# SandroMartens/DBGSOM

Hardware: NVIDIA B200
Metric: training samples/sec/epoch (higher is better)
Workload: dtype f16 tensor cores (tcgen05) + f64 re-score / f64 update / f64 smoothing

## Files before the change

### dbgsom_b200/_native.py

```python

from __future__ import annotations

import ctypes as C
import os

_LIB = None
LIB_NAME = "libdbgsom_b200.so"
LIB_PATH = os.path.join(os.path.dirname(os.path.abspath(__file__)), LIB_NAME)

ABI_VERSION = 10
COLSTATS_PARTS = 256
SELECT_OFF, SELECT_FLAG, SELECT_REFINE = 0, 1, 2
MAX_CAND = 8
BMU_SIMT = 0
BMU_TENSOR = 1
HOPS_MAX_M = 28000

c_void_p, c_int, c_int32, c_int64, c_size_t, c_float, c_double = (
    C.c_void_p, C.c_int, C.c_int32, C.c_int64, C.c_size_t, C.c_float, C.c_double,
)


class BmuArgs(C.Structure):
    _fields_ = [
        ("d_X", c_void_p),
# ... 88 lines not shown
        [c_void_p, c_int64, c_int, c_int64, c_void_p, c_float, c_void_p, c_void_p, c_int64, c_void_p, c_void_p],
    ),
    "dbgsom_prepare_x16_sorted": (
        c_int,
        [c_void_p, c_int64, c_int, c_int64, c_void_p, c_float, c_void_p, c_void_p, c_void_p, c_int64, c_void_p, c_void_p],
    ),
    "dbgsom_bmu_select_supported": (c_int, [c_int64, c_int64, c_int32, c_int32, c_int32]),
    "dbgsom_accumulate_perm_offset": (c_size_t, [c_int64, c_int32]),
    "dbgsom_prepare_w": (
        c_int,
        [c_void_p, c_int, c_int, c_void_p, c_float, c_void_p, c_void_p, c_void_p, c_int64, c_int, c_void_p,
         c_void_p, c_void_p, c_void_p, c_void_p],
    ),
    "dbgsom_exclude_duplicates": (c_int, [c_void_p, c_int, c_int, c_void_p, c_void_p, c_void_p, c_void_p]),
    "dbgsom_tile_bounds": (
        c_int, [c_void_p, c_int, c_int, c_void_p, c_float, c_void_p, c_void_p, c_int, c_void_p, c_void_p]
    ),
    "dbgsom_prepare_bias": (c_int, [c_void_p, c_int, c_void_p, c_void_p, c_void_p, c_void_p]),
    "dbgsom_bmu_workspace_bytes": (c_size_t, [c_int64, c_int32]),
    "dbgsom_bmu": (c_int, [C.POINTER(BmuArgs), c_void_p]),
    "dbgsom_bmu_candidates": (c_int, [C.POINTER(BmuArgs), c_void_p]),
    "dbgsom_bmu_resolve": (c_int, [C.POINTER(BmuArgs), c_void_p]),
    "dbgsom_accumulate_workspace_bytes": (c_size_t, [c_int64, c_int32, c_int32]),
    "dbgsom_accumulate": (c_int, [C.POINTER(AccumulateArgs), c_void_p]),
    "dbgsom_accumulate_weighted": (c_int, [C.POINTER(AccumulateArgs), c_void_p, c_void_p, c_void_p]),
    "dbgsom_smooth_workspace_bytes": (c_size_t, [c_int32, c_int32]),
    "dbgsom_smooth": (c_int, [C.POINTER(SmoothArgs), c_void_p]),
    "dbgsom_apply_row_ops": (c_int, [c_void_p, c_int, c_void_p, c_int, c_void_p]),
    "dbgsom_gather_rows": (c_int, [c_void_p, c_int64, c_int, c_void_p, c_int, c_void_p, c_void_p]),
    "dbgsom_node_stats": (
        c_int, [c_void_p, c_int32, c_void_p, c_int32, c_int64, c_void_p, c_int32, c_double, c_void_p, c_void_p]
# ... 57 lines not shown
```

### dbgsom_b200/csrc/bmu_tc.cu

```cuda
#include <cuda.h>

#include <cstdio>
#include <cstdlib>

#include "common.cuh"

namespace dbgsom {

namespace {

constexpr int BM = 128;
constexpr int BK = 64;
constexpr int UMMA_K = 16;
constexpr int A_TILE_BYTES = BM * BK * 2;
constexpr int EPI_WARP0 = 4;
constexpr int EPI_SUBS = 4;
constexpr int EPI_WARPS = 4 * EPI_SUBS;
constexpr int EPI_THREADS = EPI_WARPS * 32;
constexpr int TC_THREADS = (EPI_WARP0 + EPI_WARPS) * 32;
constexpr int KSUB = 4;
constexpr int MAX_RES_KB = 4;
constexpr int kFlagMaxCols = 4096;
constexpr int kFlagChunkBytes = kFlagMaxCols / 32 * BM * 4;

// ... 265 lines not shown
  static constexpr int RING_STAGE_BYTES = STAGES * STAGE_UNIT;
  static constexpr int SMEM_BYTES = RES_BYTES + RING_STAGE_BYTES + RING_BYTES + MISC_BYTES + WN_BYTES + EXTRA_BYTES + 1024;
  static constexpr int TMEM_COLS = ATM ? 512 : NACC * BN;
  static_assert(STAGES >= 2, "not enough shared memory for a pipeline");
};

struct Barriers {
  uint64_t full[16], empty[16];
  uint64_t a_full, a_empty;
  uint64_t tmem_full[4], tmem_empty[4];
  uint32_t tmem_base;
  EpiConst epi;
};

constexpr float kTileBoundFloor = 0.125f;
template <int NPASS, int NB, int BN, int RES_KB, int AKB, int CL, bool PAIR = false, int SEL = 0, bool TB = false,
          int SGT = 0>
__global__ void __launch_bounds__(TC_THREADS, 1)
    bmu_cand_tensor_kernel(const __grid_constant__ CUtensorMap map_xh, const __grid_constant__ CUtensorMap map_xl,
                           const __grid_constant__ CUtensorMap map_wh, const __grid_constant__ CUtensorMap map_wl,
                           const __grid_constant__ CUtensorMap map_wb, const float* __restrict__ bias_scale,
                           int64_t N, int KB, int NT, const float* __restrict__ wnorm,
                           const int32_t* __restrict__ proto_of_col, int pstride, int ties_any,
                           const float* __restrict__ xnorm16,
                           const float* __restrict__ wmax, float bound_coef, float acc_coef,
                           int32_t* __restrict__ idx_out, int32_t* __restrict__ cand_idx,
                           uint8_t* __restrict__ cand_count, const int32_t* __restrict__ row_perm,
                           unsigned long long* __restrict__ tile_mask,
                           int fg_shift, unsigned long long* __restrict__ sel_stats,
                           const float* __restrict__ tile_bound) {
// ... 383 lines not shown
    }
    const uint32_t epi_const_addr = smem_u32(&bars->epi);
    constexpr int CHUNKS = BN / 32;
    constexpr float kInf = 3.0e38f;
    if (sub == 0) row_min[t] = kInf;
    const int mpad = NT * BN;
    const bool wn_in_smem = !bias_mode && C::WN_SMEM_FLOATS > 0 && mpad <= C::WN_SMEM_FLOATS;
    if (wn_in_smem)
      for (int i = threadIdx.x - EPI_WARP0 * 32; i < mpad; i += EPI_THREADS) wn_smem[i] = wnorm[i];
    const float* wn_src = wn_in_smem ? wn_smem : wnorm;
    asm volatile("bar.sync 1, %0;" ::"n"(EPI_THREADS));
    uint32_t acc = 0, acc_phase = 0;
    uint32_t eph = 0;
    (void)eph;
    if constexpr (SEL == 1) {
      uint32_t* cta_mask = reinterpret_cast<uint32_t*>(sub_state);
      float* sub_min = reinterpret_cast<float*>(sub_state) + 4;
      if (threadIdx.x == EPI_WARP0 * 32) cta_mask[0] = cta_mask[1] = 0u;
      asm volatile("bar.sync 1, %0;" ::"n"(EPI_THREADS));
      const int n_chunks = NT * CHUNKS;
      for (int64_t it = 0; it < n_iters; ++it) {
        const int64_t row = tile_of(it) * BM + t;
        const bool valid = row < N;
        const int64_t orow = valid ? (row_perm ? (int64_t)row_perm[row] : row) : 0;
        const float tau = valid ? 2.f * tensor_score_bound(xnorm16[orow], wmax, bound_coef, acc_coef) : 0.f;
        float m1 = kInf;
        for (int nt = 0; nt < NT; ++nt) {
          mbar_wait(&bars->tmem_full[acc], acc_phase);
          tc_fence_after();
          const uint32_t tmem_acc = tmem_base + lane_base + acc * BN;
#pragma unroll 1
          for (int c = (sub - nt * CHUNKS) & (EPI_SUBS - 1); c < CHUNKS; c += EPI_SUBS) {
            uint32_t r[32];
            tmem_ld_32x32(tmem_acc + c * 32, r);
            float a1;
            if (bias_mode) {
              tmem_ld_wait();
              float gmx[8];
#pragma unroll
              for (int g = 0; g < 8; ++g)
                gmx[g] = fmaxf(fmaxf(__uint_as_float(r[4 * g + 0]), __uint_as_float(r[4 * g + 1])),
// ... 9 lines not shown
              tmem_ld_wait();
              float gmn[8];
#pragma unroll
              for (int g = 0; g < 8; ++g) {
                const float s0 = fmaf(-2.f, __uint_as_float(r[4 * g + 0]), w4[g].x);
                const float s1 = fmaf(-2.f, __uint_as_float(r[4 * g + 1]), w4[g].y);
                const float s2 = fmaf(-2.f, __uint_as_float(r[4 * g + 2]), w4[g].z);
                const float s3 = fmaf(-2.f, __uint_as_float(r[4 * g + 3]), w4[g].w);
                gmn[g] = fminf(fminf(s0, s1), fminf(s2, s3));
              }
              a1 = fminf(fminf(fminf(gmn[0], gmn[1]), fminf(gmn[2], gmn[3])),
                         fminf(fminf(gmn[4], gmn[5]), fminf(gmn[6], gmn[7])));
            }
            chunk_min[(nt * CHUNKS + c) * BM + t] = a1;
            m1 = fminf(m1, a1);
          }
          tc_fence_before();
          __syncwarp();
          if (lane == 0) mbar_arrive_cluster(mapa_u32(smem_u32(&bars->tmem_empty[acc]), 0));
          if (++acc == NACC) {
            acc = 0;
            acc_phase ^= 1;
          }
        }
        sub_min[t * EPI_SUBS + sub] = m1;
        asm volatile("bar.sync 1, %0;" ::"n"(EPI_THREADS));
        const float4 sm4 = *reinterpret_cast<const float4*>(sub_min + t * EPI_SUBS);
        const float thr = fminf(fminf(sm4.x, sm4.y), fminf(sm4.z, sm4.w)) + tau;
        uint32_t mlo = 0u, mhi = 0u;
        if (valid) {
          for (int ch = sub; ch < n_chunks; ch += EPI_SUBS) {
            const uint32_t bit = (uint32_t)(ch * 32) >> fg_shift;
            const uint32_t inb = chunk_min[ch * BM + t] <= thr ? 1u : 0u;
            mlo |= bit < 32u ? inb << bit : 0u;
            mhi |= bit >= 32u ? inb << (bit - 32u) : 0u;
          }
        }
        mlo = __reduce_or_sync(kFullMask, mlo);
        mhi = __reduce_or_sync(kFullMask, mhi);
        if (lane == 0) {
          if (mlo) atomicOr(&cta_mask[0], mlo);
          if (mhi) atomicOr(&cta_mask[1], mhi);
        }
        asm volatile("bar.sync 1, %0;" ::"n"(EPI_THREADS));
        if (threadIdx.x == EPI_WARP0 * 32) {
          const unsigned long long m64 = (unsigned long long)cta_mask[0] | ((unsigned long long)cta_mask[1] << 32);
          const int64_t pr = pair_of(it);
          if (m64 && pr < n_pairs) atomicOr(tile_mask + pr, m64);
          cta_mask[0] = cta_mask[1] = 0u;
        }
        asm volatile("bar.sync 1, %0;" ::"n"(EPI_THREADS));
      }
    } else {
    auto fetch_orow = [&](int64_t it_) -> int64_t {
      const int64_t r_ = it_ < n_iters ? tile_of(it_) * BM + t : N;
      return r_ < N ? (row_perm ? (int64_t)row_perm[r_] : r_) : -1;
    };
    auto fetch_mask = [&](int64_t it_) -> unsigned long long { return it_ < n_iters ? sel_mask(it_) : 0ull; };
    int64_t orow_n1 = fetch_orow(0);
    int64_t orow_n2 = fetch_orow(1);
    float xn_n1 = orow_n1 >= 0 ? xnorm16[orow_n1] : 0.f;
    unsigned long long mask_n1 = fetch_mask(0);
    for (int64_t it = 0; it < n_iters; ++it) {
      const int64_t row = tile_of(it) * BM + t;
      const int64_t orow = orow_n1 >= 0 ? orow_n1 : 0;
      const float tau = row < N ? 2.f * tensor_score_bound(xn_n1, wmax, bound_coef, acc_coef) : 0.f;
      const float xn_row = row < N ? xn_n1 : 0.f;
      unsigned long long selm = mask_n1;
      orow_n1 = orow_n2;
      xn_n1 = orow_n1 >= 0 ? xnorm16[orow_n1] : 0.f;
      orow_n2 = fetch_orow(it + 2);
      mask_n1 = fetch_mask(it + 1);
      float m1 = kInf, m2 = kInf, thr = kInf, evicted = __int_as_float(0x7f800000);
      float gate = __int_as_float(0x7f800000);
      asm volatile("st.shared.v4.f32 [%0], {%1,%1,%1,%1};" ::"r"(my_val_addr), "f"(gate) : "memory");
      asm volatile("st.shared.v4.s32 [%0], {%1,%1,%1,%1};" ::"r"(my_idx_addr), "r"(0x7fffffff) : "memory");
      const int n_sel = SEL == 2 ? __popcll(selm) : NT;
      for (int ti = 0; ti < n_sel; ++ti) {
        int nt = ti;
        if (SEL == 2) {
          nt = __ffsll((long long)selm) - 1;
          selm &= selm - 1;
        }
        float kb = 0.f;
        if (TB) {
          const float* tb = tile_bound + 2 * (nt * (BN / 128));
          float um = tb[0], wm = tb[1];
#pragma unroll
          for (int q = 1; q < BN / 128; ++q) {
            um = fmaxf(um, tb[2 * q]);
            wm = fmaxf(wm, tb[2 * q + 1]);
          }
          um = fmaxf(um, kTileBoundFloor * wmax[0]);
          wm = fmaxf(wm, kTileBoundFloor * wmax[2]);
          const float xw = xn_row * um;
          kb = xw * bound_coef + acc_coef * (xw + wm);
        }
// ... 24 lines not shown
              for (int e = 0; e < 16; ++e) {
                q0[e] = __float_as_uint(__uint_as_float(q0[e]) + __uint_as_float(p0[e]));
                q1[e] = __float_as_uint(__uint_as_float(q1[e]) + __uint_as_float(p1[e]));
              }
              tmem_st_32x16(qa, q0);
              tmem_st_32x16(qa + 16, q1);
            }
            tmem_st_wait();
          }
        } else {
          mbar_wait(&bars->tmem_full[acc], acc_phase);
        }
        tc_fence_after();
        const uint32_t tmem_acc = tmem_base + lane_base + acc * BN;
#pragma unroll 1
        for (int c = (sub - ti * CHUNKS) & (EPI_SUBS - 1); c < CHUNKS; c += EPI_SUBS) {
          uint32_t r[32];
          if (SEGM) {
            float sum[32];
            const int nseg = (KB + SEG - 1) / SEG;
            for (int seg = 0; seg < nseg; ++seg) {
              if (seg > 0) {
                mbar_wait(&bars->tmem_full[acc], acc_phase);
                tc_fence_after();
              }
              tmem_ld_32x32(tmem_base + lane_base + acc * BN + c * 32, r);
              tmem_ld_wait();
#pragma unroll
              for (int e = 0; e < 32; ++e) sum[e] = seg == 0 ? __uint_as_float(r[e]) : sum[e] + __uint_as_float(r[e]);
              if (seg < nseg - 1) {
                tc_fence_before();
// ... 295 lines not shown
      }
    }
    if (max_grid > (int64_t)max_clusters * CL) max_grid = (int64_t)max_clusters * CL;
  }
  if (grid > max_grid) grid = max_grid;
  cfg.gridDim = dim3((unsigned)grid);
  const float coef = tensor_bound_coef(NPASS, a.bound_scale);
  const float acc_coef = tensor_acc_coef_args(a);
  const int pstride = a.proto_stride > 0 && a.Mpad <= 65535 && a.proto_stride < a.Mpad ? a.proto_stride : 0;
  DBGSOM_CUDA_TRY(cudaLaunchKernelEx(&cfg, kern, mxh, mxl, mwh, mwl, mwb, with_bias ? a.d_bias_scale : (const float*)nullptr,
                                     a.N, KB, NT, a.d_wnorm, a.d_proto_of_col, pstride,
                                     a.n_bmu == 1 ? a.ties_any : 0, a.d_xnorm16, a.d_wmax, coef, acc_coef, a.d_idx, ws.cand_idx, ws.cand_count,
                                     a.d_row_perm, reinterpret_cast<unsigned long long*>(a.d_tile_mask),
                                     a.select_granule == 64 ? 6 : 7,
                                     a.d_stats ? reinterpret_cast<unsigned long long*>(a.d_stats) + 4 : (unsigned long long*)nullptr,
                                     TB ? a.d_tile_bound : (const float*)nullptr));
  DBGSOM_LAUNCH_CHECK();
  return DBGSOM_OK;
}

int cluster_size() {
  static int cl = 0;
  if (cl == 0) {
    const char* e = getenv("DBGSOM_TC_CLUSTER");
    cl = e ? atoi(e) : 2;
    if (cl != 1 && cl != 2 && cl != 4) cl = 2;
  }
  return cl;
}

template <int NPASS, int NB, int BN, int RES_KB, int AKB = 0>
// ... 19 lines not shown
  static const bool pairs = getenv("DBGSOM_TC_PAIR") == nullptr || atoi(getenv("DBGSOM_TC_PAIR")) != 0;
  return a.backend == DBGSOM_BMU_TENSOR && a.n_pass == 3 && a.ld16 / BK > MAX_RES_KB && pairs && cluster_size() >= 2 &&
         ceil_div<int64_t>(a.N, BM) >= sm_count();
}
int streamed_segm_mode() {
  static const int mode = getenv("DBGSOM_TC_SEGM") == nullptr ? 3 : atoi(getenv("DBGSOM_TC_SEGM"));
  return mode;
}
bool streamed_segmented(const dbgsom_bmu_args& a) { return streamed_segm_mode() == 1 && streamed_pairs(a); }
int streamed_tmem_sums(const dbgsom_bmu_args& a) {
  const int mode = streamed_segm_mode();
  return (mode == 2 || mode == 3) && streamed_pairs(a) ? (mode == 2 ? 8 : 4) : 0;
}
}
bool tile_bounds_active(const dbgsom_bmu_args& a) {
  return a.d_tile_bound != nullptr && a.n_bmu == 1 && a.select == DBGSOM_SELECT_OFF && streamed_pairs(a);
}
namespace {

template <int NPASS, int NB>
int launch_shape(const dbgsom_bmu_args& a, const BmuWorkspace& ws, cudaStream_t s) {
  const int KB = (int)(a.ld16 / BK);
  if constexpr (NPASS == 1) {
    if (KB <= 2) return launch_cfg<NPASS, NB, 256, 2>(a, ws, s);
    if (KB <= MAX_RES_KB) return launch_cfg<NPASS, NB, 256, 4>(a, ws, s);
    return launch_cfg<NPASS, NB, 256, 0>(a, ws, s);
  } else {
    static const bool a_smem = getenv("DBGSOM_TC_A_SMEM") != nullptr;
    if (KB <= 2) return a_smem ? launch_cfg<NPASS, NB, 128, 2>(a, ws, s) : launch_cfg<NPASS, NB, 128, 0, 2>(a, ws, s);
    if (KB <= MAX_RES_KB)
      return a_smem ? launch_cfg<NPASS, NB, 128, 4>(a, ws, s) : launch_cfg<NPASS, NB, 128, 0, 4>(a, ws, s);
// ... 80 lines not shown
```

### dbgsom_b200/csrc/capi.cu

```cuda
#include "common.cuh"

namespace dbgsom {
int run_colstats(const float*, int64_t, int, int64_t, const float*, const double*, double*, cudaStream_t);
int run_prepare_x16(const float*, int64_t, int, int64_t, const float*, float, const int32_t*, uint16_t*, uint16_t*, int64_t,
                    float*, cudaStream_t);
size_t accumulate_perm_offset(int64_t, int);
bool bmu_select_supported(int64_t N, int64_t ld16, int Mpad, int n_bmu, int granule);
int run_prepare_w(const double*, int, int, const float*, float, float*, uint16_t*, uint16_t*, int64_t, int,
                  const int32_t*, float*, double*, float*, cudaStream_t);
int run_exclude_duplicates(const double*, int, int, const int32_t*, float*, unsigned long long*, cudaStream_t);
int run_tile_bounds(const double*, int, int, const double*, float, const int32_t*, const float*, int, float*, cudaStream_t);
int run_prepare_bias(const float*, int, const float*, uint16_t*, float*, cudaStream_t);
int run_row_ops(double*, int, const int32_t*, int, cudaStream_t);
int run_gather_rows(const float*, int64_t, int, const int64_t*, int, double*, cudaStream_t);
size_t accumulate_workspace_bytes(int64_t, int, int);
int run_accumulate(const dbgsom_accumulate_args&, const double*, double*, cudaStream_t);
size_t label_hist_weighted_workspace_bytes(int64_t, int);
int run_label_counts_weighted(const int32_t*, const int32_t*, const double*, int64_t, int, int, double*, void*, cudaStream_t);
size_t smooth_workspace_bytes(int, int);
int run_smooth(const dbgsom_smooth_args&, cudaStream_t);
int run_node_stats(const int32_t*, int, const double*, int, int64_t, const int32_t*, int, double, const double*, double*,
                   cudaStream_t);
int run_label_hist(const int32_t*, int, const int32_t*, const double*, int64_t, int64_t, int, int, int32_t*, int64_t*,
                   cudaStream_t);
int run_umatrix(const double*, int, int, int64_t, const double*, double*, cudaStream_t);
int run_hops(const int32_t*, int, uint16_t*, int64_t, cudaStream_t);
// ... 97 lines not shown
  }
  if (a->D % 4 != 0 || a->ldx % 4 != 0 || !aligned16(a->d_X) || !aligned16(a->d_W32) || !aligned16(a->d_W))
    return DBGSOM_E_UNSUPPORTED;
  if (a->workspace_bytes < BmuWorkspace::bytes(a->N)) return DBGSOM_E_WORKSPACE;
  return DBGSOM_OK;
}

int dbgsom_exclude_duplicates(const double* d_W, int M, int D, const int32_t* d_col_of_proto, float* d_wnorm,
                              uint64_t* d_hash, void* stream) {
  if (!d_W || !d_wnorm || !d_hash || M <= 0 || D <= 0) return DBGSOM_E_BADARG;
  return run_exclude_duplicates(d_W, M, D, d_col_of_proto, d_wnorm, reinterpret_cast<unsigned long long*>(d_hash),
                                as_stream(stream));
}

int dbgsom_tile_bounds(const double* d_W, int M, int D, const double* d_wshift, float scale,
                       const int32_t* d_proto_of_col, const float* d_wnorm, int Mpad, float* d_tile_bound, void* stream) {
  if (!d_W || !d_wshift || !d_wnorm || !d_tile_bound || M <= 0 || D <= 0 || Mpad < M) return DBGSOM_E_BADARG;
  if (Mpad % 128 != 0) return DBGSOM_E_UNSUPPORTED;
  return run_tile_bounds(d_W, M, D, d_wshift, scale, d_proto_of_col, d_wnorm, Mpad, d_tile_bound, as_stream(stream));
}

int dbgsom_prepare_bias(const float* d_wnorm, int Mpad, const float* d_wmax, uint16_t* d_Wb16, float* d_bias_scale,
                        void* stream) {
  if (!d_wnorm || !d_wmax || !d_Wb16 || !d_bias_scale || Mpad <= 0) return DBGSOM_E_BADARG;
  return run_prepare_bias(d_wnorm, Mpad, d_wmax, d_Wb16, d_bias_scale, as_stream(stream));
}

int dbgsom_bmu_candidates(const dbgsom_bmu_args* a, void* stream) {
  const int rc = check_bmu_args(a);
  if (rc != DBGSOM_OK) return rc;
  const BmuWorkspace ws = BmuWorkspace::carve(a->d_workspace, a->N);
  if (a->backend == DBGSOM_BMU_SIMT) return launch_bmu_cand_simt(*a, ws, as_stream(stream));
  return launch_bmu_cand_tensor(*a, ws, as_stream(stream));
}
// ... 128 lines not shown
```

### dbgsom_b200/csrc/common.cuh

```cuda
#pragma once

#include <cuda_fp16.h>
#include <cuda_runtime.h>
#include <stdint.h>

#include <cmath>
#include <cstdlib>

#include "../../include/dbgsom_b200.h"

#define DBGSOM_CUDA_TRY(expr)                  \
  do {                                         \
    cudaError_t _e = (expr);                   \
    if (_e != cudaSuccess) return (int)_e;     \
  } while (0)

#define DBGSOM_LAUNCH_CHECK()                  \
  do {                                         \
    cudaError_t _e = cudaGetLastError();       \
    if (_e != cudaSuccess) return (int)_e;     \
  } while (0)

namespace dbgsom {

// ... 145 lines not shown
  }
};

__device__ __forceinline__ float tensor_score_bound(float xnorm, const float* __restrict__ wmax, float coef, float acc_coef) {
  const float xw = xnorm * wmax[0];
  return xw * coef + acc_coef * (xw + wmax[2]);
}
inline float tensor_acc_coef(int n_pass, int64_t ld16, int strict) {
  const double steps = (double)(ld16 / 16) * (n_pass == 3 ? 3.0 : 1.0);
  double c = 2.4e-7 * (steps > 48.0 ? (strict ? steps / 48.0 : sqrt(steps / 48.0)) : 1.0);
  if (const char* e = getenv("DBGSOM_ACC_SCALE")) c *= atof(e);
  return (float)c;
}
float tensor_acc_coef_args(const dbgsom_bmu_args& a);
bool tile_bounds_active(const dbgsom_bmu_args& a);
__host__ __device__ inline float tensor_bound_coef(int n_pass, float bound_scale) {
  if (n_pass == 1) return (bound_scale > 0.f ? bound_scale : 0.25f) * 1.953125e-3f;
  return (bound_scale > 0.f ? bound_scale : 0.0625f) * 1.9073486e-6f;
}

struct BmuWorkspace {
  int32_t* cand_idx;
  uint8_t* cand_count;
  int32_t* rescan_count;
  int32_t* rescan_rows;
  __host__ static size_t bytes(int64_t N) {
    return round_up<size_t>((size_t)N * kMaxCand * sizeof(int32_t), 256) + round_up<size_t>((size_t)N, 256) + 256 +
           round_up<size_t>((size_t)N * sizeof(int32_t), 256);
  }
  __host__ static BmuWorkspace carve(void* base, int64_t N) {
// ... 19 lines not shown
```

### dbgsom_b200/csrc/prep.cu

```cuda
#include "common.cuh"

namespace dbgsom {

namespace {

constexpr int CS_COLS = 32, CS_ROWS = 8;
template <bool WGT>
__global__ void __launch_bounds__(CS_COLS * CS_ROWS) colstats_kernel(const float* __restrict__ X, int64_t N, int D,
                                                                    int64_t ldx, const float* __restrict__ shift,
                                                                    const double* __restrict__ weight,
                                                                    double* __restrict__ moments,
                                                                    int64_t rows_per_block) {
  __shared__ double s1[CS_ROWS][CS_COLS], s2[CS_ROWS][CS_COLS], s3[CS_ROWS][CS_COLS];
  const int cx = threadIdx.x % CS_COLS, ry = threadIdx.x / CS_COLS;
  const int d = blockIdx.x * CS_COLS + cx;
  const int64_t r0 = (int64_t)blockIdx.y * rows_per_block;
  const int64_t r1 = r0 + rows_per_block < N ? r0 + rows_per_block : N;
  double a1 = 0.0, a2 = 0.0, a3 = 0.0;
  if (d < D) {
    const float c = shift[d];
    for (int64_t r = r0 + ry; r < r1; r += CS_ROWS) {
      const double t = (double)X[r * ldx + d] - (double)c;
      const double wt = WGT ? weight[r] * t : t;
      a1 += wt;
// ... 123 lines not shown
    nr = red[1][0] + red[1][1] + red[1][2] + red[1][3];
    uv = red[2][0] + red[2][1] + red[2][2] + red[2][3];
    const double bias = nu + 2.0 * uv;
    if (wnorm) wnorm[col] = j < M ? (float)bias : __int_as_float(0x7f800000);
    if (j < M) {
      atomicMax(reinterpret_cast<int*>(wmax + 0), __float_as_int(__double2float_ru(sqrt(nu))));
      atomicMax(reinterpret_cast<int*>(wmax + 1), __float_as_int(__double2float_ru(sqrt(nr))));
      atomicMax(reinterpret_cast<int*>(wmax + 2), __float_as_int(__double2float_ru(fabs(bias))));
    }
  }
}

__global__ void __launch_bounds__(256) tile_bounds_kernel(const double* __restrict__ W, int M, int D,
                                                         const double* __restrict__ wshift, float scale,
                                                         const int32_t* __restrict__ proto_of_col,
                                                         const float* __restrict__ wnorm, float* __restrict__ out) {
  __shared__ float red[2][8];
  const int lane = threadIdx.x & 31, warp = threadIdx.x >> 5;
  float um = 0.f, wm = 0.f;
  for (int i = warp; i < 128; i += 8) {
    const int c = blockIdx.x * 128 + i;
    const int j = proto_of_col ? proto_of_col[c] : c;
    const float wn = wnorm[c];
    if (j < 0 || j >= M || !(fabsf(wn) < 3.0e38f)) continue;
    double nu = 0.0;
    for (int d = lane; d < D; d += 32) {
      const double u = (W[(int64_t)j * D + d] - wshift[d]) * (double)scale;
      nu = fma(u, u, nu);
    }
    nu = warp_sum(nu);
    um = fmaxf(um, __double2float_ru(sqrt(nu)));
    wm = fmaxf(wm, fabsf(wn));
  }
  if (lane == 0) {
    red[0][warp] = um;
    red[1][warp] = wm;
// ... 145 lines not shown
  DBGSOM_CUDA_TRY(cudaMemsetAsync(wmax, 0, 4 * sizeof(float), s));
  if (W16_hi) {
    if (!wshift) return DBGSOM_E_BADARG;
    w_colmean_kernel<<<ceil_div(D, 32), 256, 0, s>>>(W, M, D, wshift);
    DBGSOM_LAUNCH_CHECK();
  }
  const int rows = W16_hi ? (Mpad > M ? Mpad : M) : M;
  prepare_w_kernel<<<rows, 128, 0, s>>>(W, M, D, shift, wshift, scale, W32, reinterpret_cast<__half*>(W16_hi),
                                        reinterpret_cast<__half*>(W16_lo), ld16, W16_hi ? col_of_proto : nullptr, wnorm,
                                        wmax);
  DBGSOM_LAUNCH_CHECK();
  return DBGSOM_OK;
}

int run_tile_bounds(const double* W, int M, int D, const double* wshift, float scale, const int32_t* proto_of_col,
                    const float* wnorm, int Mpad, float* out, cudaStream_t s) {
  tile_bounds_kernel<<<Mpad / 128, 256, 0, s>>>(W, M, D, wshift, scale, proto_of_col, wnorm, out);
  DBGSOM_LAUNCH_CHECK();
  return DBGSOM_OK;
}

int run_exclude_duplicates(const double* W, int M, int D, const int32_t* col_of_proto, float* wnorm,
                           unsigned long long* hash, cudaStream_t s) {
  row_hash_kernel<<<M, 128, 0, s>>>(W, M, D, hash);
  DBGSOM_LAUNCH_CHECK();
  mark_duplicates_kernel<<<ceil_div(M, 256), 256, 0, s>>>(W, M, D, hash, col_of_proto, wnorm);
  DBGSOM_LAUNCH_CHECK();
  return DBGSOM_OK;
}

int run_prepare_bias(const float* wnorm, int Mpad, const float* wmax, uint16_t* Wb16, float* bias_scale, cudaStream_t s) {
  bias_rows_kernel<<<ceil_div(Mpad, 256), 256, 0, s>>>(wnorm, Mpad, wmax, reinterpret_cast<__half*>(Wb16), bias_scale);
// ... 20 lines not shown
```

### dbgsom_b200/engine.py

```python

from __future__ import annotations

import math
import os
from typing import Sequence

import numpy as np

from . import _native as nat
from . import streaming
from .hostmath import class_entropy, column_moments_to_stats

_UPLOAD_ROWS = 1 << 20


def scatter_stride(mpad: int) -> int:
    stride = int(round(mpad * 0.6180339887498949)) | 1
    while math.gcd(stride, mpad) != 1:
        stride += 2
    return stride


def _round_up(a: int, b: int) -> int:
    return (a + b - 1) // b * b
# ... 583 lines not shown
                proto_of_col = np.random.default_rng(0x5EED + mpad).permutation(mpad).astype(np.int32)
                stride = 0
            if os.environ.get("DBGSOM_PERM") == "table":
                stride = 0
        col_of_proto = np.empty_like(proto_of_col)
        col_of_proto[proto_of_col] = np.arange(mpad, dtype=np.int32)
        hit = (torch.from_numpy(proto_of_col).to(self.dev), torch.from_numpy(col_of_proto).to(self.dev), stride)
        if len(self._perm_cache) > 8:
            self._perm_cache.clear()
        self._perm_cache[key] = hit
        return hit

    def _prepare_w(self, W, m: int, tensor: bool, need_lo: bool, top1: bool = True, map_order: bool = False) -> int:
        torch = self.torch
        mpad = _round_up(m, 256)
        tile = bool(tensor and need_lo and top1 and self.tile_bounds_enabled and self.ld16 > 256)
        if tile and self._map_order is not None and len(self._map_order) == m:
            map_order = True
        self._tile_ready = False
        if tensor:
            self.proto_of_col, self.col_of_proto, self.proto_stride = self._column_order(m, mpad, map_order)
            if self.W16_hi is None or self.W16_hi.shape[0] < mpad or (need_lo and self.W16_lo is None):
                rows = _round_up(max(mpad, self.cap), 256)
                self.W16_hi = torch.zeros((rows, self.ld16), dtype=torch.float16, device=self.dev)
                self.W16_lo = torch.zeros((rows, self.ld16), dtype=torch.float16, device=self.dev) if need_lo else None
                self.wnorm = torch.empty(rows, dtype=torch.float32, device=self.dev)
                self.Wb16 = torch.zeros((rows, 64), dtype=torch.float16, device=self.dev)
                self.bias_scale = torch.zeros(1, dtype=torch.float32, device=self.dev)
        nat.check(
            self.lib.dbgsom_prepare_w(
                W.data_ptr(), m, self.ldx, self.shift.data_ptr(), self.scale, self.W32.data_ptr(),
                self.W16_hi.data_ptr() if tensor else None,
# ... 6 lines not shown
        )
        self.launches += 3 if tensor else 2
        self._ties_any = bool(tensor and top1)
        if self._ties_any:
            if getattr(self, "_row_hash", None) is None or self._row_hash.numel() < m:
                self._row_hash = torch.empty(max(m, self.cap), dtype=torch.int64, device=self.dev)
            nat.check(
                self.lib.dbgsom_exclude_duplicates(
                    W.data_ptr(), m, self.ldx, self.col_of_proto.data_ptr(), self.wnorm.data_ptr(),
                    self._row_hash.data_ptr(), self._stream(),
                ),
                "dbgsom_exclude_duplicates",
            )
            self.launches += 2
        if tile:
            if self.tile_bound is None or self.tile_bound.numel() < mpad // 64:
                self.tile_bound = torch.zeros(_round_up(max(mpad, self.cap), 256) // 64, dtype=torch.float32, device=self.dev)
            nat.check(
                self.lib.dbgsom_tile_bounds(W.data_ptr(), m, self.ldx, self.wshift.data_ptr(), self.scale,
                                            self.proto_of_col.data_ptr(), self.wnorm.data_ptr(), mpad,
                                            self.tile_bound.data_ptr(), self._stream()),
                "dbgsom_tile_bounds",
            )
            self.launches += 1
            self._tile_ready = True
        flag_bias = bool(tensor and need_lo and top1 and map_order and not tile and self.ld16 <= 128
                         and os.environ.get("DBGSOM_FLAG_BIAS", "0") == "1")
        self._flag_bias_ready = False
        if flag_bias or (tensor and need_lo and os.environ.get("DBGSOM_TC_BIAS", "0") == "1"):
            nat.check(
                self.lib.dbgsom_prepare_bias(self.wnorm.data_ptr(), mpad, self.wmax.data_ptr(), self.Wb16.data_ptr(),
                                             self.bias_scale.data_ptr(), self._stream()),
                "dbgsom_prepare_bias",
            )
            self.launches += 1
            self._bias_ready = os.environ.get("DBGSOM_TC_BIAS", "0") == "1"
            self._flag_bias_ready = flag_bias
        else:
            self._bias_ready = False
        return mpad

# ... 23 lines not shown
        ws_bytes = self.lib.dbgsom_bmu_workspace_bytes(n, n_bmu)
        ws = self._workspace(ws_key, ws_bytes)
        a = nat.BmuArgs()
        a.d_X, a.N, a.D, a.ldx, a.ld16 = X.data_ptr(), n, self.ldx, ldx, self.ld16
        if tensor:
            xh, xl, xn = x16
            a.d_X16_hi, a.d_X16_lo, a.d_xnorm16 = xh.data_ptr(), (xl.data_ptr() if xl is not None else None), xn.data_ptr()
            a.d_W16_hi = self.W16_hi.data_ptr()
            a.d_W16_lo = self.W16_lo.data_ptr() if self.W16_lo is not None else None
            a.d_wnorm = self.wnorm.data_ptr()
            if getattr(self, "_bias_ready", False):
                a.d_Wb16, a.d_bias_scale = self.Wb16.data_ptr(), self.bias_scale.data_ptr()
            a.d_proto_of_col = self.proto_of_col.data_ptr()
            a.proto_stride = self.proto_stride
            a.ties_any = int(self._ties_any and n_bmu == 1)
            if self._tile_ready and n_bmu == 1 and n_pass == 3 and not selective:
                a.d_tile_bound = self.tile_bound.data_ptr()
        a.d_W, a.d_W32, a.d_wmax = W.data_ptr(), self.W32.data_ptr(), self.wmax.data_ptr()
        a.scale, a.M, a.Mpad, a.n_bmu = self.scale, m, mpad, n_bmu
        a.backend, a.n_pass, a.bound_scale, a.tie_rel = be, n_pass, self.bound_scale, 0.0
        a.strict, a.want_dist = int(self.strict_ties if strict is None else strict), int(want_dist)
        a.d_idx, a.d_dist = idx.data_ptr(), (dist.data_ptr() if dist is not None else None)
        a.d_stats = self.bmu_stats.data_ptr()
        a.d_workspace, a.workspace_bytes = ws.data_ptr(), ws.numel()
        if tensor and row_perm is not None:
            a.d_row_perm = row_perm.data_ptr()
        if selective:
            n_pairs = -(-(-(-n // 128)) // 2)
            if self.tile_mask is None or self.tile_mask.numel() < n_pairs:
                self.tile_mask = self.torch.zeros(n_pairs, dtype=self.torch.int64, device=self.dev)
            self.tile_mask.zero_()
            a.d_tile_mask = self.tile_mask.data_ptr()
            a.select_granule = self.select_granule
            a.select, a.n_pass = nat.SELECT_FLAG, 1
            if getattr(self, "_flag_bias_ready", False):
                a.d_Wb16, a.d_bias_scale = self.Wb16.data_ptr(), self.bias_scale.data_ptr()
            with self._Phase(self, "bmu_candidates"):
                nat.check(self.lib.dbgsom_bmu_candidates(a, self._stream()), "dbgsom_bmu_candidates[flag]")
            a.d_Wb16, a.d_bias_scale = None, None
            a.select, a.n_pass = nat.SELECT_REFINE, 3
            with self._Phase(self, "bmu_second_stage"):
                nat.check(self.lib.dbgsom_bmu_candidates(a, self._stream()), "dbgsom_bmu_candidates[refine]")
            self.launches += 2
            self._epoch_kinds["selective"] += 1
        else:
            if tensor and n_pass == 3 and n_bmu == 1:
# ... 561 lines not shown
```

### include/dbgsom_b200.h

```cpp
#ifndef DBGSOM_B200_H
#define DBGSOM_B200_H

#include <stddef.h>
#include <stdint.h>

#ifdef __cplusplus
extern "C" {
#endif

#define DBGSOM_ABI_VERSION 10

#define DBGSOM_OK 0
#define DBGSOM_E_BADARG (-1)
#define DBGSOM_E_WORKSPACE (-2)
#define DBGSOM_E_UNSUPPORTED (-3)
#define DBGSOM_E_DRIVER (-4)
#define DBGSOM_E_NOT_SM100 (-5)

#define DBGSOM_MAX_CAND 8
#define DBGSOM_CAND_OVERFLOW 255
#define DBGSOM_HOP_INF 0xFFFFu

#define DBGSOM_BMU_SIMT 0
#define DBGSOM_BMU_TENSOR 1

// ... 13 lines not shown

int dbgsom_prepare_x16_sorted(const float* d_X, int64_t N, int D, int64_t ldx, const float* d_shift, float scale,
                              const int32_t* d_perm, uint16_t* d_X16_hi, uint16_t* d_X16_lo, int64_t ld16,
                              float* d_xnorm16, void* stream);

int dbgsom_prepare_w(const double* d_W, int M, int D, const float* d_shift, float scale, float* d_W32,
                     uint16_t* d_W16_hi, uint16_t* d_W16_lo, int64_t ld16, int Mpad,
                     const int32_t* d_col_of_proto , float* d_wnorm ,
                     double* d_wshift , float* d_wmax , void* stream);

int dbgsom_exclude_duplicates(const double* d_W, int M, int D, const int32_t* d_col_of_proto ,
                              float* d_wnorm, uint64_t* d_hash, void* stream);

int dbgsom_tile_bounds(const double* d_W, int M, int D, const double* d_wshift , float scale,
                       const int32_t* d_proto_of_col , const float* d_wnorm , int Mpad,
                       float* d_tile_bound , void* stream);

int dbgsom_prepare_bias(const float* d_wnorm, int Mpad, const float* d_wmax, uint16_t* d_Wb16 ,
                        float* d_bias_scale , void* stream);

typedef struct dbgsom_bmu_args {
  const float* d_X;
  const uint16_t* d_X16_hi;
  const uint16_t* d_X16_lo;
  const float* d_xnorm16;
  int64_t N;
  int32_t D;
  int64_t ldx;
  int64_t ld16;
  const double* d_W;
  const float* d_W32;
// ... 121 lines not shown
```

Measured before the change: 326.3 million.

## Tighten flag-pass tile selection with per-tile score bounds

```diff
diff --git a/dbgsom_b200/_native.py b/dbgsom_b200/_native.py
--- a/dbgsom_b200/_native.py
+++ b/dbgsom_b200/_native.py
@@ -8,7 +8,7 @@
 LIB_NAME = "libdbgsom_b200.so"
 LIB_PATH = os.path.join(os.path.dirname(os.path.abspath(__file__)), LIB_NAME)
 
-ABI_VERSION = 10
+ABI_VERSION = 11
 COLSTATS_PARTS = 256
 SELECT_OFF, SELECT_FLAG, SELECT_REFINE = 0, 1, 2
 MAX_CAND = 8
@@ -127,7 +127,7 @@
     ),
     "dbgsom_exclude_duplicates": (c_int, [c_void_p, c_int, c_int, c_void_p, c_void_p, c_void_p, c_void_p]),
     "dbgsom_tile_bounds": (
-        c_int, [c_void_p, c_int, c_int, c_void_p, c_float, c_void_p, c_void_p, c_int, c_void_p, c_void_p]
+        c_int, [c_void_p, c_int, c_int, c_void_p, c_float, c_void_p, c_void_p, c_int, c_int, c_void_p, c_void_p]
     ),
     "dbgsom_prepare_bias": (c_int, [c_void_p, c_int, c_void_p, c_void_p, c_void_p, c_void_p]),
     "dbgsom_bmu_workspace_bytes": (c_size_t, [c_int64, c_int32]),
diff --git a/dbgsom_b200/csrc/bmu_tc.cu b/dbgsom_b200/csrc/bmu_tc.cu
--- a/dbgsom_b200/csrc/bmu_tc.cu
+++ b/dbgsom_b200/csrc/bmu_tc.cu
@@ -303,6 +303,12 @@
 };
 
 constexpr float kTileBoundFloor = 0.125f;
+__device__ __forceinline__ float tile_score_bound(float xnorm, const float* __restrict__ tb, float ufloor, float wfloor,
+                                                  float coef, float acc_coef) {
+  const float2 t = *reinterpret_cast<const float2*>(tb);
+  const float xw = xnorm * fmaxf(t.x, ufloor);
+  return xw * coef + acc_coef * (xw + fmaxf(t.y, wfloor));
+}
 template <int NPASS, int NB, int BN, int RES_KB, int AKB, int CL, bool PAIR = false, int SEL = 0, bool TB = false,
           int SGT = 0>
 __global__ void __launch_bounds__(TC_THREADS, 1)
@@ -716,17 +722,21 @@
     uint32_t eph = 0;
     (void)eph;
     if constexpr (SEL == 1) {
+      const bool per_tile = tile_bound != nullptr && !bias_mode;
+      const float ufloor = kTileBoundFloor * wmax[0], wfloor = kTileBoundFloor * wmax[2];
       uint32_t* cta_mask = reinterpret_cast<uint32_t*>(sub_state);
       float* sub_min = reinterpret_cast<float*>(sub_state) + 4;
-      if (threadIdx.x == EPI_WARP0 * 32) cta_mask[0] = cta_mask[1] = 0u;
+      float* sub_ub = sub_min + BM * EPI_SUBS;
+      if (threadIdx.x == EPI_WARP0 * 32) cta_mask[0] = cta_mask[1] = cta_mask[2] = cta_mask[3] = 0u;
       asm volatile("bar.sync 1, %0;" ::"n"(EPI_THREADS));
       const int n_chunks = NT * CHUNKS;
       for (int64_t it = 0; it < n_iters; ++it) {
         const int64_t row = tile_of(it) * BM + t;
         const bool valid = row < N;
         const int64_t orow = valid ? (row_perm ? (int64_t)row_perm[row] : row) : 0;
-        const float tau = valid ? 2.f * tensor_score_bound(xnorm16[orow], wmax, bound_coef, acc_coef) : 0.f;
-        float m1 = kInf;
+        const float xn = valid ? xnorm16[orow] : 0.f;
+        const float tau = valid ? 2.f * tensor_score_bound(xn, wmax, bound_coef, acc_coef) : 0.f;
+        float m1 = kInf, u1 = kInf;
         for (int nt = 0; nt < NT; ++nt) {
           mbar_wait(&bars->tmem_full[acc], acc_phase);
           tc_fence_after();
@@ -766,6 +776,10 @@
             }
             chunk_min[(nt * CHUNKS + c) * BM + t] = a1;
             m1 = fminf(m1, a1);
+            if (per_tile) {
+              const float* tb = tile_bound + 2 * ((uint32_t)(nt * BN + c * 32) >> fg_shift);
+              u1 = fminf(u1, a1 + tile_score_bound(xn, tb, ufloor, wfloor, bound_coef, acc_coef));
+            }
           }
           tc_fence_before();
           __syncwarp();
@@ -776,16 +790,28 @@
           }
         }
         sub_min[t * EPI_SUBS + sub] = m1;
+        if (per_tile) sub_ub[t * EPI_SUBS + sub] = u1;
         asm volatile("bar.sync 1, %0;" ::"n"(EPI_THREADS));
         const float4 sm4 = *reinterpret_cast<const float4*>(sub_min + t * EPI_SUBS);
         const float thr = fminf(fminf(sm4.x, sm4.y), fminf(sm4.z, sm4.w)) + tau;
-        uint32_t mlo = 0u, mhi = 0u;
+        float U = kInf;
+        if (per_tile) {
+          const float4 su4 = *reinterpret_cast<const float4*>(sub_ub + t * EPI_SUBS);
+          U = fminf(fminf(su4.x, su4.y), fminf(su4.z, su4.w));
+        }
+        uint32_t mlo = 0u, mhi = 0u, wlo = 0u, whi = 0u;
         if (valid) {
           for (int ch = sub; ch < n_chunks; ch += EPI_SUBS) {
             const uint32_t bit = (uint32_t)(ch * 32) >> fg_shift;
-            const uint32_t inb = chunk_min[ch * BM + t] <= thr ? 1u : 0u;
+            const float cm = chunk_min[ch * BM + t];
+            const bool wide = cm <= thr;
+            const bool in = wide && (!per_tile ||
+                                     cm - tile_score_bound(xn, tile_bound + 2 * bit, ufloor, wfloor, bound_coef, acc_coef) <= U);
+            const uint32_t inb = in ? 1u : 0u, wnb = wide ? 1u : 0u;
             mlo |= bit < 32u ? inb << bit : 0u;
             mhi |= bit >= 32u ? inb << (bit - 32u) : 0u;
+            wlo |= bit < 32u ? wnb << bit : 0u;
+            whi |= bit >= 32u ? wnb << (bit - 32u) : 0u;
           }
         }
         mlo = __reduce_or_sync(kFullMask, mlo);
@@ -794,12 +820,22 @@
           if (mlo) atomicOr(&cta_mask[0], mlo);
           if (mhi) atomicOr(&cta_mask[1], mhi);
         }
+        if (per_tile) {
+          wlo = __reduce_or_sync(kFullMask, wlo);
+          whi = __reduce_or_sync(kFullMask, whi);
+          if (lane == 0) {
+            if (wlo) atomicOr(&cta_mask[2], wlo);
+            if (whi) atomicOr(&cta_mask[3], whi);
+          }
+        }
         asm volatile("bar.sync 1, %0;" ::"n"(EPI_THREADS));
         if (threadIdx.x == EPI_WARP0 * 32) {
           const unsigned long long m64 = (unsigned long long)cta_mask[0] | ((unsigned long long)cta_mask[1] << 32);
+          const unsigned long long w64 = (unsigned long long)cta_mask[2] | ((unsigned long long)cta_mask[3] << 32);
           const int64_t pr = pair_of(it);
           if (m64 && pr < n_pairs) atomicOr(tile_mask + pr, m64);
-          cta_mask[0] = cta_mask[1] = 0u;
+          if (w64 && pr < n_pairs) atomicOr(tile_mask + n_pairs + pr, w64);
+          cta_mask[0] = cta_mask[1] = cta_mask[2] = cta_mask[3] = 0u;
         }
         asm volatile("bar.sync 1, %0;" ::"n"(EPI_THREADS));
       }
@@ -809,20 +845,27 @@
       return r_ < N ? (row_perm ? (int64_t)row_perm[r_] : r_) : -1;
     };
     auto fetch_mask = [&](int64_t it_) -> unsigned long long { return it_ < n_iters ? sel_mask(it_) : 0ull; };
+    const bool wide_rot = SEL == 2 && tile_bound != nullptr;
+    auto fetch_wide = [&](int64_t it_) -> unsigned long long {
+      const int64_t pr = pair_of(it_);
+      return wide_rot && it_ < n_iters && pr < n_pairs ? tile_mask[n_pairs + pr] : 0ull;
+    };
     int64_t orow_n1 = fetch_orow(0);
     int64_t orow_n2 = fetch_orow(1);
     float xn_n1 = orow_n1 >= 0 ? xnorm16[orow_n1] : 0.f;
-    unsigned long long mask_n1 = fetch_mask(0);
+    unsigned long long mask_n1 = fetch_mask(0), wide_n1 = fetch_wide(0);
     for (int64_t it = 0; it < n_iters; ++it) {
       const int64_t row = tile_of(it) * BM + t;
       const int64_t orow = orow_n1 >= 0 ? orow_n1 : 0;
       const float tau = row < N ? 2.f * tensor_score_bound(xn_n1, wmax, bound_coef, acc_coef) : 0.f;
       const float xn_row = row < N ? xn_n1 : 0.f;
       unsigned long long selm = mask_n1;
+      const unsigned long long widem = wide_n1;
       orow_n1 = orow_n2;
       xn_n1 = orow_n1 >= 0 ? xnorm16[orow_n1] : 0.f;
       orow_n2 = fetch_orow(it + 2);
       mask_n1 = fetch_mask(it + 1);
+      wide_n1 = fetch_wide(it + 1);
       float m1 = kInf, m2 = kInf, thr = kInf, evicted = __int_as_float(0x7f800000);
       float gate = __int_as_float(0x7f800000);
       asm volatile("st.shared.v4.f32 [%0], {%1,%1,%1,%1};" ::"r"(my_val_addr), "f"(gate) : "memory");
@@ -830,9 +873,11 @@
       const int n_sel = SEL == 2 ? __popcll(selm) : NT;
       for (int ti = 0; ti < n_sel; ++ti) {
         int nt = ti;
+        int rot = ti;
         if (SEL == 2) {
           nt = __ffsll((long long)selm) - 1;
           selm &= selm - 1;
+          if (wide_rot) rot = __popcll(widem & ((1ull << nt) - 1ull));
         }
         float kb = 0.f;
         if (TB) {
@@ -887,7 +932,7 @@
         tc_fence_after();
         const uint32_t tmem_acc = tmem_base + lane_base + acc * BN;
 #pragma unroll 1
-        for (int c = (sub - ti * CHUNKS) & (EPI_SUBS - 1); c < CHUNKS; c += EPI_SUBS) {
+        for (int c = (sub - rot * CHUNKS) & (EPI_SUBS - 1); c < CHUNKS; c += EPI_SUBS) {
           uint32_t r[32];
           if (SEGM) {
             float sum[32];
@@ -1213,7 +1258,7 @@
                                      a.d_row_perm, reinterpret_cast<unsigned long long*>(a.d_tile_mask),
                                      a.select_granule == 64 ? 6 : 7,
                                      a.d_stats ? reinterpret_cast<unsigned long long*>(a.d_stats) + 4 : (unsigned long long*)nullptr,
-                                     TB ? a.d_tile_bound : (const float*)nullptr));
+                                     TB || (SEL != 0 && flag_tile_bounds(a)) ? a.d_tile_bound : (const float*)nullptr));
   DBGSOM_LAUNCH_CHECK();
   return DBGSOM_OK;
 }
@@ -1263,7 +1308,11 @@
 }
 }
 bool tile_bounds_active(const dbgsom_bmu_args& a) {
-  return a.d_tile_bound != nullptr && a.n_bmu == 1 && a.select == DBGSOM_SELECT_OFF && streamed_pairs(a);
+  return a.d_tile_bound != nullptr && a.n_bmu == 1 &&
+         (a.select == DBGSOM_SELECT_FLAG || (a.select == DBGSOM_SELECT_OFF && streamed_pairs(a)));
+}
+bool flag_tile_bounds(const dbgsom_bmu_args& a) {
+  return a.d_tile_bound != nullptr && a.n_bmu == 1 && a.select != DBGSOM_SELECT_OFF;
 }
 namespace {
 
diff --git a/dbgsom_b200/csrc/capi.cu b/dbgsom_b200/csrc/capi.cu
--- a/dbgsom_b200/csrc/capi.cu
+++ b/dbgsom_b200/csrc/capi.cu
@@ -9,7 +9,7 @@
 int run_prepare_w(const double*, int, int, const float*, float, float*, uint16_t*, uint16_t*, int64_t, int,
                   const int32_t*, float*, double*, float*, cudaStream_t);
 int run_exclude_duplicates(const double*, int, int, const int32_t*, float*, unsigned long long*, cudaStream_t);
-int run_tile_bounds(const double*, int, int, const double*, float, const int32_t*, const float*, int, float*, cudaStream_t);
+int run_tile_bounds(const double*, int, int, const double*, float, const int32_t*, const float*, int, int, float*, cudaStream_t);
 int run_prepare_bias(const float*, int, const float*, uint16_t*, float*, cudaStream_t);
 int run_row_ops(double*, int, const int32_t*, int, cudaStream_t);
 int run_gather_rows(const float*, int64_t, int, const int64_t*, int, double*, cudaStream_t);
@@ -137,10 +137,12 @@
 }
 
 int dbgsom_tile_bounds(const double* d_W, int M, int D, const double* d_wshift, float scale,
-                       const int32_t* d_proto_of_col, const float* d_wnorm, int Mpad, float* d_tile_bound, void* stream) {
+                       const int32_t* d_proto_of_col, const float* d_wnorm, int Mpad, int granule, float* d_tile_bound,
+                       void* stream) {
   if (!d_W || !d_wshift || !d_wnorm || !d_tile_bound || M <= 0 || D <= 0 || Mpad < M) return DBGSOM_E_BADARG;
-  if (Mpad % 128 != 0) return DBGSOM_E_UNSUPPORTED;
-  return run_tile_bounds(d_W, M, D, d_wshift, scale, d_proto_of_col, d_wnorm, Mpad, d_tile_bound, as_stream(stream));
+  if ((granule != 64 && granule != 128) || Mpad % granule != 0) return DBGSOM_E_UNSUPPORTED;
+  return run_tile_bounds(d_W, M, D, d_wshift, scale, d_proto_of_col, d_wnorm, Mpad, granule, d_tile_bound,
+                         as_stream(stream));
 }
 
 int dbgsom_prepare_bias(const float* d_wnorm, int Mpad, const float* d_wmax, uint16_t* d_Wb16, float* d_bias_scale,
diff --git a/dbgsom_b200/csrc/common.cuh b/dbgsom_b200/csrc/common.cuh
--- a/dbgsom_b200/csrc/common.cuh
+++ b/dbgsom_b200/csrc/common.cuh
@@ -183,6 +183,7 @@
 }
 float tensor_acc_coef_args(const dbgsom_bmu_args& a);
 bool tile_bounds_active(const dbgsom_bmu_args& a);
+bool flag_tile_bounds(const dbgsom_bmu_args& a);
 __host__ __device__ inline float tensor_bound_coef(int n_pass, float bound_scale) {
   if (n_pass == 1) return (bound_scale > 0.f ? bound_scale : 0.25f) * 1.953125e-3f;
   return (bound_scale > 0.f ? bound_scale : 0.0625f) * 1.9073486e-6f;
diff --git a/dbgsom_b200/csrc/prep.cu b/dbgsom_b200/csrc/prep.cu
--- a/dbgsom_b200/csrc/prep.cu
+++ b/dbgsom_b200/csrc/prep.cu
@@ -161,12 +161,13 @@
 __global__ void __launch_bounds__(256) tile_bounds_kernel(const double* __restrict__ W, int M, int D,
                                                          const double* __restrict__ wshift, float scale,
                                                          const int32_t* __restrict__ proto_of_col,
-                                                         const float* __restrict__ wnorm, float* __restrict__ out) {
+                                                         const float* __restrict__ wnorm, int granule,
+                                                         float* __restrict__ out) {
   __shared__ float red[2][8];
   const int lane = threadIdx.x & 31, warp = threadIdx.x >> 5;
   float um = 0.f, wm = 0.f;
-  for (int i = warp; i < 128; i += 8) {
-    const int c = blockIdx.x * 128 + i;
+  for (int i = warp; i < granule; i += 8) {
+    const int c = blockIdx.x * granule + i;
     const int j = proto_of_col ? proto_of_col[c] : c;
     const float wn = wnorm[c];
     if (j < 0 || j >= M || !(fabsf(wn) < 3.0e38f)) continue;
@@ -342,8 +343,8 @@
 }
 
 int run_tile_bounds(const double* W, int M, int D, const double* wshift, float scale, const int32_t* proto_of_col,
-                    const float* wnorm, int Mpad, float* out, cudaStream_t s) {
-  tile_bounds_kernel<<<Mpad / 128, 256, 0, s>>>(W, M, D, wshift, scale, proto_of_col, wnorm, out);
+                    const float* wnorm, int Mpad, int granule, float* out, cudaStream_t s) {
+  tile_bounds_kernel<<<Mpad / granule, 256, 0, s>>>(W, M, D, wshift, scale, proto_of_col, wnorm, granule, out);
   DBGSOM_LAUNCH_CHECK();
   return DBGSOM_OK;
 }
diff --git a/dbgsom_b200/engine.py b/dbgsom_b200/engine.py
--- a/dbgsom_b200/engine.py
+++ b/dbgsom_b200/engine.py
@@ -621,8 +621,10 @@
     def _prepare_w(self, W, m: int, tensor: bool, need_lo: bool, top1: bool = True, map_order: bool = False) -> int:
         torch = self.torch
         mpad = _round_up(m, 256)
-        tile = bool(tensor and need_lo and top1 and self.tile_bounds_enabled and self.ld16 > 256)
-        if tile and self._map_order is not None and len(self._map_order) == m:
+        streamed = self.ld16 > 256
+        tile = bool(tensor and need_lo and top1 and self.tile_bounds_enabled and (streamed or map_order))
+        granule = 128 if streamed else self.select_granule
+        if tile and streamed and self._map_order is not None and len(self._map_order) == m:
             map_order = True
         self._tile_ready = False
         if tensor:
@@ -659,17 +661,17 @@
             )
             self.launches += 2
         if tile:
-            if self.tile_bound is None or self.tile_bound.numel() < mpad // 64:
-                self.tile_bound = torch.zeros(_round_up(max(mpad, self.cap), 256) // 64, dtype=torch.float32, device=self.dev)
+            if self.tile_bound is None or self.tile_bound.numel() < 2 * mpad // granule:
+                self.tile_bound = torch.zeros(_round_up(max(mpad, self.cap), 256) // 32, dtype=torch.float32, device=self.dev)
             nat.check(
                 self.lib.dbgsom_tile_bounds(W.data_ptr(), m, self.ldx, self.wshift.data_ptr(), self.scale,
-                                            self.proto_of_col.data_ptr(), self.wnorm.data_ptr(), mpad,
+                                            self.proto_of_col.data_ptr(), self.wnorm.data_ptr(), mpad, granule,
                                             self.tile_bound.data_ptr(), self._stream()),
                 "dbgsom_tile_bounds",
             )
             self.launches += 1
             self._tile_ready = True
-        flag_bias = bool(tensor and need_lo and top1 and map_order and not tile and self.ld16 <= 128
+        flag_bias = bool(tensor and need_lo and top1 and map_order and self.ld16 <= 128
                          and os.environ.get("DBGSOM_FLAG_BIAS", "0") == "1")
         self._flag_bias_ready = False
         if flag_bias or (tensor and need_lo and os.environ.get("DBGSOM_TC_BIAS", "0") == "1"):
@@ -723,7 +725,7 @@
             a.d_proto_of_col = self.proto_of_col.data_ptr()
             a.proto_stride = self.proto_stride
             a.ties_any = int(self._ties_any and n_bmu == 1)
-            if self._tile_ready and n_bmu == 1 and n_pass == 3 and not selective:
+            if self._tile_ready and n_bmu == 1 and n_pass == 3:
                 a.d_tile_bound = self.tile_bound.data_ptr()
         a.d_W, a.d_W32, a.d_wmax = W.data_ptr(), self.W32.data_ptr(), self.wmax.data_ptr()
         a.scale, a.M, a.Mpad, a.n_bmu = self.scale, m, mpad, n_bmu
@@ -736,9 +738,9 @@
             a.d_row_perm = row_perm.data_ptr()
         if selective:
             n_pairs = -(-(-(-n // 128)) // 2)
-            if self.tile_mask is None or self.tile_mask.numel() < n_pairs:
-                self.tile_mask = self.torch.zeros(n_pairs, dtype=self.torch.int64, device=self.dev)
-            self.tile_mask.zero_()
+            if self.tile_mask is None or self.tile_mask.numel() < 2 * n_pairs:
+                self.tile_mask = self.torch.zeros(2 * n_pairs, dtype=self.torch.int64, device=self.dev)
+            self.tile_mask[: 2 * n_pairs].zero_()
             a.d_tile_mask = self.tile_mask.data_ptr()
             a.select_granule = self.select_granule
             a.select, a.n_pass = nat.SELECT_FLAG, 1
diff --git a/include/dbgsom_b200.h b/include/dbgsom_b200.h
--- a/include/dbgsom_b200.h
+++ b/include/dbgsom_b200.h
@@ -8,7 +8,7 @@
 extern "C" {
 #endif
 
-#define DBGSOM_ABI_VERSION 10
+#define DBGSOM_ABI_VERSION 11
 
 #define DBGSOM_OK 0
 #define DBGSOM_E_BADARG (-1)
@@ -52,7 +52,7 @@
 
 int dbgsom_tile_bounds(const double* d_W, int M, int D, const double* d_wshift , float scale,
                        const int32_t* d_proto_of_col , const float* d_wnorm , int Mpad,
-                       float* d_tile_bound , void* stream);
+                       int granule, float* d_tile_bound , void* stream);
 
 int dbgsom_prepare_bias(const float* d_wnorm, int Mpad, const float* d_wmax, uint16_t* d_Wb16 ,
                         float* d_bias_scale , void* stream);
```

Measured after the change: 322.6 million (median of 6 runs). 0.989x the previous value.
